# ndjinga/CirculantPreconditioner

Hardware: AMD Instinct MI355X
Metric: PCApply/s on 256^3 complex grid (higher is better)
Workload: dtype c128 (f64 complex); 1 GPU; 256x256x256 c128 circulant PCApply, transport symbol lambda=(0.6, 0.15, 0.02); global_batch=1, parallelism=single GPU

## Files before the change

### circulantpreconditioner_amd/_lib_ext.py

```python
from __future__ import annotations

import ctypes


class PetscScalar(ctypes.Structure):
    _fields_ = [("re", ctypes.c_double), ("im", ctypes.c_double)]

    @classmethod
    def of(cls, v) -> "PetscScalar":
        c = complex(v)
        return cls(c.real, c.imag)

    def __complex__(self):
        return complex(self.re, self.im)


class FFTPrecTransportContext(ctypes.Structure):
    _fields_ = [("spaceDim", ctypes.c_int64), ("n_x", ctypes.c_int64), ("n_y", ctypes.c_int64),
                ("n_z", ctypes.c_int64), ("lambda_x", PetscScalar), ("lambda_y", PetscScalar),
                ("lambda_z", PetscScalar), ("FFT_MAT", ctypes.c_void_p), ("intersectionMatrix", ctypes.c_void_p),
                ("Diag", ctypes.c_void_p), ("b_hat", ctypes.c_void_p), ("b_cartesien", ctypes.c_void_p)]


class StructuredTransportContext(ctypes.Structure):
# ... 42 lines not shown

class WaveResult(ctypes.Structure):
    _fields_ = [("steps", ctypes.c_int64), ("dt", ctypes.c_double), ("time", ctypes.c_double),
                ("total_its", ctypes.c_int64), ("max_step_its", ctypes.c_int64), ("min_step_its", ctypes.c_int64),
                ("last_reason", ctypes.c_int), ("all_converged", ctypes.c_int), ("last_residual", ctypes.c_double),
                ("last_norm_dU", ctypes.c_double), ("solve_seconds", ctypes.c_double),
                ("pc_seconds", ctypes.c_double), ("pc_calls", ctypes.c_int64), ("setup_seconds", ctypes.c_double),
                ("kappa", ctypes.c_double * 3), ("rstart", ctypes.c_int64), ("nlocal", ctypes.c_int64),
                ("loop_seconds", ctypes.c_double), ("dev_ms_", ctypes.c_double * 4),
                ("dev_launches_", ctypes.c_int64 * 4), ("fused_dots", ctypes.c_int64), ("fused_norms", ctypes.c_int64)]

    def as_dict(self) -> dict:
        d = {k: getattr(self, k) for k, _ in self._fields_ if k != "kappa" and not k.endswith("_")}
        d["kappa"] = list(self.kappa)
        d["dev_ms"] = dict(zip(("pcapply", "matmult", "vector", "copy"), self.dev_ms_))
        d["dev_launches"] = dict(zip(("pcapply", "matmult", "vector", "copy"), self.dev_launches_))
        return d


def declare(L) -> None:
    i64, dp, vp, c_int = ctypes.c_int64, ctypes.c_void_p, ctypes.c_void_p, ctypes.c_int
    S, P, cs = PetscScalar, ctypes.POINTER, ctypes.c_char_p
    sig = {
        "cfp_dist_get_unique_id": ([ctypes.c_char_p], c_int),
        "cfp_dist_unique_id_bytes": ([], c_int),
        "cfp_slab_layout": ([i64, i64, i64, c_int, c_int, P(i64)], c_int),
        "cfp_slab_work_size": ([i64, i64, i64, c_int, c_int, P(i64)], c_int),
        "cfp_slab_num_steps": ([i64, i64, i64, c_int, c_int, P(c_int)], c_int),
        "cfp_slab_step_info": ([i64, i64, i64, c_int, c_int, c_int, P(i64), P(ctypes.c_double)], c_int),
        "cfp_dist_plan_create": ([P(vp), i64, i64, i64, c_int, c_int, ctypes.c_char_p, c_int], c_int),
        "cfp_dist_plan_create_timeout": ([P(vp), i64, i64, i64, c_int, c_int, ctypes.c_char_p, c_int,
                                          ctypes.c_double], c_int),
        "cfp_dist_plan_rccl_info": ([vp, P(c_int), P(c_int), P(c_int), P(ctypes.c_double), ctypes.c_char_p, c_int],
                                    c_int),
        "cfp_rccl_version": ([P(c_int), ctypes.c_char_p, c_int], c_int),
        "cfp_rccl_blocking": ([P(c_int)], c_int),
        "cfp_dist_plan_destroy": ([vp], c_int),
        "cfp_dist_plan_create_external": ([P(vp), i64, i64, i64, c_int, c_int, c_int], c_int),
        "cfp_dist_plan_work_buffer": ([vp, P(ctypes.c_void_p)], c_int),
        "cfp_dist_plan_run_segment": ([vp, c_int, dp, dp, vp], c_int),
        "cfp_dist_plan_set_work_buffer": ([vp, dp], c_int),
        "cfp_dist_plan_set_symbol_transport": ([vp, dp], c_int),
        "cfp_dist_plan_apply": ([vp, dp, dp, vp], c_int),
        "cfp_dist_plan_profile_begin": ([vp, c_int, c_int], c_int),
        "cfp_dist_plan_profile_end": ([vp, dp, P(c_int)], c_int),
        "cfp_dist_plan_local_size": ([vp, P(i64)], c_int),
# ... 195 lines not shown
```

### circulantpreconditioner_amd/csrc/cfp_plan.hip

```cpp
#include <hip/hip_runtime.h>

#include <cmath>
#include <complex>
#include <cstdio>
#include <cstring>
#include <map>
#include <memory>
#include <mutex>
#include <string>
#include <vector>

#include "../../include/circulant_fft.h"
#include "cfp_blas.h"
#include "cfp_internal.h"
#include "cfp_host.h"
#include "cfp_three_pass.h"

using namespace cfp;

static thread_local std::string g_err;

namespace cfp {
int set_error(int code, const char* fmt, ...) {
  char buf[512];
// ... 35 lines not shown
  return CFP_SUCCESS;
}

namespace cfp {

std::vector<cd> host_twiddles(int n, int sign) {
  std::vector<cd> t((size_t)n);
  for (int k = 0; k < n; ++k) {
    long double a = 2.0L * 3.14159265358979323846264338327950288L * (long double)k / (long double)n;
    t[k] = make_cd((double)cosl(a), (double)(sign * sinl(a)));
  }
  return t;
}

std::vector<cd> host_transport_symbol(i64 n) {
  std::vector<cd> s((size_t)n, make_cd(0.0, 0.0));
  if (n <= 1) return s;
  for (i64 k = 0; k < n; ++k) {
    long double a = 2.0L * 3.14159265358979323846264338327950288L * (long double)k / (long double)n;
    s[k] = make_cd((double)(1.0L - cosl(a)), (double)sinl(a));
  }
  return s;
}

int ilog2_exact(i64 v) {
  if (v <= 0 || (v & (v - 1))) return -1;
  int l = 0;
  while ((1LL << l) < v) ++l;
  return l;
}

Side natural_side(int axis, const i64 n[3]) {
  Side s;
  const i64 nx = n[0], ny = n[1];
  s.seg_len = (int)n[axis];
  s.seg_shift = ilog2_exact(n[axis]);
  if (s.seg_shift < 0) s.seg_shift = 30;
  s.seg_stride = 0;
  if (axis == 0) { s.inner_stride = 0; s.outer_stride = nx; s.pt_stride = 1; }
  else if (axis == 1) { s.inner_stride = 1; s.outer_stride = nx * ny; s.pt_stride = nx; }
  else { s.inner_stride = 1; s.outer_stride = 0; s.pt_stride = nx * ny; }
  if (ilog2_exact(n[axis]) < 0) s.seg_shift = -1;
  return s;
}

void natural_cols(int axis, const i64 n[3], i64* ncols, i64* inner_n) {
// ... 12 lines not shown
  int sym_kind = 0;
  uint64_t sym_version = 0;
  cd* colsym = nullptr;
  cd* axsym = nullptr;
  cd* diag = nullptr;
  cd* host_stage = nullptr;
  cd* mid_buf = nullptr;
  double* post_partial = nullptr;
  cd* pre_buf = nullptr;
  struct GraphEntry {
    const cd* b;
    cd* x;
    hipGraphExec_t exec;
  };
  bool graph_on = false;
  hipStream_t cap_stream = nullptr;
  std::vector<GraphEntry> graphs;
  std::vector<int> axes;
  int fused_axis = 0;
  std::vector<cd> sym1d[3];
  i64 chunk_planes = 0;
  int schedule = CFP_SCHEDULE_AUTO;
  TPShape tp_shape;
  bool external_x = false;
  int split[3][2] = {{0, 0}, {0, 0}, {0, 0}};
  cd* tw4lo[3] = {nullptr, nullptr, nullptr};
  cd* tw4hi[3] = {nullptr, nullptr, nullptr};
  cd* possym[3] = {nullptr, nullptr, nullptr};
  bool long_axes() const { return split[0][0] || split[1][0] || split[2][0]; }
  std::vector<hipEvent_t> prof_ev;
  size_t prof_stride = 0, prof_cap = 0, prof_used = 0;
  size_t prof_every = 1, prof_calls = 0;
};

namespace cfp {
thread_local LaunchStamp g_stamp;
thread_local ApplyStamp g_apply_stamp;
}
extern "C" void cfp_apply_stamp_clear(void) { cfp::g_apply_stamp.start = cfp::g_apply_stamp.stop = nullptr; }

namespace {

struct DeviceGuard {
  int prev = -1;
  explicit DeviceGuard(int dev) {
    hipGetDevice(&prev);
// ... 12 lines not shown
  cd* d = nullptr;
  HIPCHK(hipMalloc(&d, sizeof(cd) * (size_t)n));
  HIPCHK(hipMemcpy(d, h.data(), sizeof(cd) * (size_t)n, hipMemcpyHostToDevice));
  p->tw[n] = d;
  return CFP_SUCCESS;
}

struct Step {
  int axis;
  int mode;
  bool from_b;
  bool scale;
  i64 z0, z1;
  int tp = -1;
  int sub = 0;
};

bool use_three_pass(const cfp_plan_s* p, bool diag_override) {
  const bool want = p->schedule == CFP_SCHEDULE_THREE_PASS ||
                    (p->schedule == CFP_SCHEDULE_AUTO && p->chunk_planes == 0 &&
                     (p->n[0] == 256 || p->n[0] == 128 || p->n[0] == 100 || p->n[0] == 512));
  if (!want || diag_override || p->sym_kind != 1 || p->external_x) return false;
  return three_pass_supported(p->n) || three_pass_sq_supported(p->n);
}

bool use_plane(const cfp_plan_s* p) {
  if (p->external_x || p->long_axes() || p->n[0] != p->n[1] || !plane_supported(p->n[0]) || p->n[2] < 2)
    return false;
  if (p->schedule == CFP_SCHEDULE_PLANE) return true;
  return p->schedule == CFP_SCHEDULE_AUTO && p->chunk_planes == 0 &&
         (p->n[0] == 100 || p->n[0] == 64 || p->n[0] == 32);
}

void order_axes(cfp_plan_s* p) {
  p->axes.clear();
  const int order_z[3] = {0, 1, 2}, order_y[3] = {0, 2, 1};
  const bool yf = p->schedule == CFP_SCHEDULE_FIVE_PASS_YFUSED ||
                  (p->schedule == CFP_SCHEDULE_AUTO && p->n[1] >= 512 && p->n[2] >= 512 && !three_pass_supported(p->n));
  const int* o = (yf && !p->long_axes()) ? order_y : order_z;
  std::vector<int> longs;
  for (int i = 0; i < 3; ++i) {
    if (p->n[o[i]] <= 1 || (p->external_x && o[i] == 0)) continue;
    if (p->split[o[i]][0]) longs.push_back(o[i]);
    else p->axes.push_back(o[i]);
  }
  p->fused_axis = p->axes.empty() ? (longs.empty() ? 0 : -1) : p->axes.back();
// ... 164 lines not shown
      if ((tn == 256 || tn == 512) && (p->tp_shape.mid == TP_MID_BLOCKED || p->tp_shape.mid == TP_MID_BLOCKED32)) {
        if (!p->mid_buf) HIPCHK(hipMalloc(&p->mid_buf, sizeof(cd) * (size_t)p->N));
        if (q.tp == 2) tin = p->mid_buf;
        else tout = p->mid_buf;
      }
      hipError_t e;
      if (fz && q.tp == 0 && fz->pre_cls) {
        a.pre_cls = fz->pre_cls;
        a.pre_cls_x = fz->pre_cls_x;
        a.pre_mask = fz->pre_mask;
        a.pre_tab = fz->pre_tab;
        a.pre_nd = fz->pre_nd;
        a.pre_ncls = fz->pre_ncls;
        for (int k = 0; k < 3; ++k) a.pre_off[k] = fz->pre_off[k];
        e = launch_three_pass_fused(0, tn, tin, tout, a, s, nullptr);
      } else if (fz && q.tp == 2 && fz->post_nv > 0) {
        for (int j = 0; j < TP_POST_MAX; ++j) a.post_v[j] = fz->post_v[j];
        a.post_nv = fz->post_nv;
        a.post_self = fz->post_self;
        a.post_partial = fz->post_partial;
        e = launch_three_pass_fused(2, tn, tin, tout, a, s, p3grid);
      } else {
        a.krylov = fz != nullptr || g_apply_stamp.start != nullptr;
        e = launch_three_pass(q.tp, tn, tin, tout, a, p->tp_shape, s);
      }
      g_stamp = LaunchStamp{};
      if (e != hipSuccess) return hip_error(e, "3-sweep launch");
      continue;
    }
    if (q.sub == 4) {
      const int pn = (int)p->n[0];
      int prc = ensure_tw(p, pn);
      if (prc) return prc;
      if (ev) HIPCHK(hipEventRecord((*ev)[2 * i], s));
      hipError_t e = launch_plane_pass(q.mode == PASS_PLANE_INV, pn, p->n[2], q.from_b ? b : x, x, p->tw[pn],
                                       q.scale ? invN : 1.0, s);
      if (e != hipSuccess) return hip_error(e, "plane pass launch");
      if (ev) HIPCHK(hipEventRecord((*ev)[2 * i + 1], s));
      continue;
    }
    if (q.sub == 3) {
      if (ev) HIPCHK(hipEventRecord((*ev)[2 * i], s));
      hipError_t e = launch_sym_divide_positions(x, p->possym[0], p->possym[1], p->possym[2], p->n[0], p->n[1],
                                                 p->n[2], s);
      if (e != hipSuccess) return hip_error(e, "symbol divide");
      if (ev) HIPCHK(hipEventRecord((*ev)[2 * i + 1], s));
// ... 102 lines not shown
  free_symbol(p);
  HIPCHK(hipMalloc(&p->colsym, sizeof(cd) * (size_t)ncols));
  HIPCHK(hipMalloc(&p->axsym, sizeof(cd) * (size_t)nf));
  HIPCHK(hipMemcpy(p->colsym, col.data(), sizeof(cd) * (size_t)ncols, hipMemcpyHostToDevice));
  HIPCHK(hipMemcpy(p->axsym, ax.data(), sizeof(cd) * (size_t)nf, hipMemcpyHostToDevice));
  for (int a = 0; a < 3; ++a) p->sym1d[a] = s_nat[a];
  p->sym_kind = 1;
  return CFP_SUCCESS;
}

int set_separable(cfp_plan_s* p, const std::vector<cd> hat[3], const double lam[6]) {
  std::vector<cd> s[3];
  for (int a = 0; a < 3; ++a) {
    std::complex<double> l = lamc(lam, a);
    s[a].resize(hat[a].size());
    for (size_t k = 0; k < hat[a].size(); ++k) {
      std::complex<double> c(hat[a][k].x, hat[a][k].y);
      const double re = c.real() * l.real() - c.imag() * l.imag();
      const double im = c.real() * l.imag() + c.imag() * l.real();
      s[a][k] = make_cd(re, im);
    }
  }
  ++p->sym_version;
  return upload_separable(p, s);
}

}

extern "C" int cfp_plan_create(cfp_plan_t* plan, int64_t nx, int64_t ny, int64_t nz, int device) {
  if (!plan) return set_error(CFP_ERR_ARG_NULL, "plan is NULL");
  *plan = nullptr;
  if (nx < 1 || ny < 1 || nz < 1) return set_error(CFP_ERR_ARG_OUTOFRANGE, "grid sizes must be >= 1");
  const int64_t dims_in[3] = {nx, ny, nz};
  int split[3][2] = {{0, 0}, {0, 0}, {0, 0}};
  for (int a = 0; a < 3; ++a) {
    if (dims_in[a] <= 4096) continue;
    i64 best = 0;
    for (i64 d = 2; d <= 4096; ++d)
      if (dims_in[a] % d == 0 && dims_in[a] / d <= 4096) {
        const i64 o = dims_in[a] / d;
        if (best == 0 || std::llabs(d - o) < std::llabs(best - dims_in[a] / best)) best = d;
      }
    if (best == 0)
      return set_error(CFP_ERR_SUP, "axis length %lld is not a product of two factors <= 4096", (long long)dims_in[a]);
    split[a][0] = (int)best;
    split[a][1] = (int)(dims_in[a] / best);
  }
  int ndev = 0;
// ... 51 lines not shown
  }
  if (p->host_stage) hipFree(p->host_stage);
  if (p->mid_buf) hipFree(p->mid_buf);
  if (p->post_partial) hipFree(p->post_partial);
  if (p->pre_buf) hipFree(p->pre_buf);
  graph_clear(p);
  if (p->cap_stream) hipStreamDestroy(p->cap_stream);
  for (auto& e : p->prof_ev) hipEventDestroy(e);
  delete p;
  return CFP_SUCCESS;
}

extern "C" int cfp_plan_symbol_version(cfp_plan_t p, uint64_t* version) {
  if (!p || !version) return set_error(CFP_ERR_ARG_NULL, "NULL argument");
  *version = p->sym_version;
  return CFP_SUCCESS;
}

extern "C" int cfp_plan_set_symbol_transport(cfp_plan_t p, const double lam[6]) {
  if (!p || !lam) return set_error(CFP_ERR_ARG_NULL, "NULL argument");
  DeviceGuard dg(p->device);
  std::vector<cd> hat[3];
  for (int a = 0; a < 3; ++a) hat[a] = host_transport_symbol(p->n[a]);
  return set_separable(p, hat, lam);
}

extern "C" int cfp_plan_set_symbol_separable(cfp_plan_t p, const double* cx, const double* cy, const double* cz,
                                             const double lam[6]) {
  if (!p || !cx || !cy || !cz || !lam) return set_error(CFP_ERR_ARG_NULL, "NULL argument");
  DeviceGuard dg(p->device);
  std::vector<cd> hat[3];
  const double* src[3] = {cx, cy, cz};
  for (int a = 0; a < 3; ++a) {
    hat[a].resize((size_t)p->n[a]);
    std::memcpy(hat[a].data(), src[a], sizeof(cd) * (size_t)p->n[a]);
  }
  return set_separable(p, hat, lam);
}

extern "C" int cfp_plan_set_diag(cfp_plan_t p, const double* diag, int on_device) {
  if (!p || !diag) return set_error(CFP_ERR_ARG_NULL, "NULL argument");
  if (p->long_axes()) return set_error(CFP_ERR_SUP, "an explicit Diag needs axes <= 4096 (use a separable symbol)");
  DeviceGuard dg(p->device);
  free_symbol(p);
  ++p->sym_version;
  HIPCHK(hipMalloc(&p->diag, sizeof(cd) * (size_t)p->N));
  HIPCHK(hipMemcpy(p->diag, diag, sizeof(cd) * (size_t)p->N, on_device ? hipMemcpyDeviceToDevice : hipMemcpyHostToDevice));
  p->sym_kind = 2;
  return CFP_SUCCESS;
}

extern "C" int cfp_plan_get_diag(cfp_plan_t p, double* diag_dev, void* stream) {
  if (!p || !diag_dev) return set_error(CFP_ERR_ARG_NULL, "NULL argument");
  DeviceGuard dg(p->device);
  hipStream_t s = (hipStream_t)stream;
  if (p->sym_kind == 2) {
    HIPCHK(hipMemcpyAsync(diag_dev, p->diag, sizeof(cd) * (size_t)p->N, hipMemcpyDeviceToDevice, s));
    return CFP_SUCCESS;
  }
  if (p->sym_kind != 1) return set_error(CFP_ERR_ARG_WRONGSTATE, "no symbol set");
  cd* tmp[3] = {nullptr, nullptr, nullptr};
  for (int a = 0; a < 3; ++a) {
    HIPCHK(hipMalloc(&tmp[a], sizeof(cd) * (size_t)p->n[a]));
    HIPCHK(hipMemcpy(tmp[a], p->sym1d[a].data(), sizeof(cd) * (size_t)p->n[a], hipMemcpyHostToDevice));
  }
  const cd one = make_cd(1.0, 0.0);
  hipError_t e = launch_build_diag_separable((cd*)diag_dev, tmp[0], tmp[1], tmp[2], p->n[0], p->n[1], p->n[2], one,
                                             one, one, s);
// ... 398 lines not shown
```

### circulantpreconditioner_amd/csrc/cfp_three_pass.h

```cpp
#pragma once
#include "cfp_internal.h"

namespace cfp {

#ifndef CFP_ROWS_XCD
#define CFP_ROWS_XCD 1
#endif

struct TPArgs {
  const cd* tw;
  const cd* colsym;
  const cd* axsym;
  double scale;
  int lnyl = 0;
  i64 chunk = 0;
  int k1_off = 0;
  const unsigned char* pre_cls = nullptr;
  const unsigned char* pre_cls_x = nullptr;
  const unsigned char* pre_mask = nullptr;
  const cd* pre_tab = nullptr;
  int pre_nd = 0, pre_ncls = 0;
  int pre_off[3] = {0, 0, 0};
  const cd* post_v[4] = {nullptr, nullptr, nullptr, nullptr};
  int post_nv = 0;
  int post_self = 0;
  double* post_partial = nullptr;
  int krylov = 0;
};


enum { TP_MID_DEFAULT = 0, TP_MID_LANE64 = 1, TP_MID_LANE32 = 2, TP_MID_SWAP64 = 3, TP_MID_SWAP64_PF = 4,
       TP_MID_BLOCKED = 5, TP_MID_BLOCKED32 = 6, TP_MID_SWAP32X = 7, TP_MID_ROWSALT = 8 };
struct TPShape {
  int n1 = 0;
  int mid = 0;
};

#define TP_PRE_MAX_CLS 16
#define TP_POST_MAX 4
bool three_pass_fused_supported(int n, TPShape shape);
hipError_t launch_three_pass_fused(int stage, int n, const cd* in, cd* out, const TPArgs& a, hipStream_t s,
                                   unsigned* grid_out);

bool three_pass_supported(const i64 n[3]);
bool three_pass_sq_supported(const i64 n[3]);
hipError_t launch_three_pass_sq(int stage, int n, const cd* in, cd* out, const TPArgs& a, TPShape shape,
                                hipStream_t s);
bool three_pass_shape_valid(int n1, int mid, i64 n = 0);
hipError_t launch_three_pass(int stage, int n, const cd* in, cd* out, const TPArgs& a, TPShape shape,
                             hipStream_t s);
bool three_pass_slab_supported(const i64 n[3], int P);
int three_pass_slab_n2(i64 n);
hipError_t launch_three_pass_slab(int stage, int n, const cd* in, cd* out, const TPArgs& a, int nzl, hipStream_t s);
hipError_t launch_three_pass_real(int stage, int n, const double* b, cd* H, cd* Q, double* x, const TPArgs& a,
                                  hipStream_t s, bool alt_rows = false);

struct WTPArgs {
  const cd* tw;
  WaveSym wave;
  double scale;
  const cd* post_v[4] = {nullptr, nullptr, nullptr, nullptr};
  int post_nv = 0, post_self = 0;
  double* post_partial = nullptr;
};
bool wave_three_pass_supported(const i64 n[3], int ncomp);
// ... 5 lines not shown
```

### circulantpreconditioner_amd/csrc/cfp_three_pass.hip

```cpp
#include "cfp_fft_device.h"
#include "cfp_lane.h"
#include "cfp_three_pass.h"

#include <hip/hip_ext.h>

#ifndef CFP_REAL_MID_XCD
#define CFP_REAL_MID_XCD 1
#endif

#define TP_LAUNCH(K, G, B, S, ...)                                                                    \
  do {                                                                                                \
    if (g_stamp.start || g_stamp.stop)                                                                \
      hipExtLaunchKernelGGL(K, G, B, 0, S, g_stamp.start, g_stamp.stop, 0, __VA_ARGS__);              \
    else                                                                                              \
      hipLaunchKernelGGL(K, G, B, 0, S, __VA_ARGS__);                                                 \
  } while (0)

namespace cfp {

namespace {

__device__ __forceinline__ cd dft4_dif(cd v, int q) {
  const cd p = dpp_c<DPP_XOR2>(v);
  cd t = (q & 2) ? csub(p, v) : cadd(v, p);
// ... 683 lines not shown
    if constexpr (PF) {
      lds_barrier();
      if (it + (int)gridDim.x < nunits) prefetch(XCD ? xcd_unit(it + gridDim.x, gridDim.x) : it + (int)gridDim.x);
    }
    stage_b(v);
    {
      const int c = idx(c0), tz = idx(tz0);
      const cd w = tw_y(u, c);
      cd* dst = col_ptr(u, c, tz);
      if constexpr (PROBE & PR_NO_STORE) {
        double acc = 0.0;
#pragma unroll
        for (int m = 0; m < 16; ++m) acc += v[m].x * w.x + v[m].y;
        if (acc == 1.2345e300) dst[0] = make_cd(acc, 0.0);
      } else {
#pragma unroll
        for (int m = 0; m < 16; ++m) gstore<ST>(dst + zs * TZ * m, cconj(cmul(v[m], w)));
      }
    }
    if constexpr (!PF) lds_barrier();
  }
}


bool three_pass_supported(const i64 n[3]) {
  return n[0] == n[1] && n[1] == n[2] && (n[0] == 128 || n[0] == 256 || n[0] == 512);
}

static int cu_count() {
  static int cus = 0;
  if (!cus) {
    int dev = 0;
    if (hipGetDevice(&dev) != hipSuccess ||
        hipDeviceGetAttribute(&cus, hipDeviceAttributeMultiprocessorCount, dev) != hipSuccess || cus < 1)
      cus = 256;
  }
  return cus;
}

static unsigned grid_of(int units, int per_cu) {
  const int g = per_cu * cu_count();
  return (unsigned)(units < g ? units : g);
}
static unsigned grid_xcd(int units, int per_cu) {
  unsigned g = grid_of(units, per_cu), p = 1;
  while (2 * p <= g) p *= 2;
// ... 276 lines not shown
  else launch_rows<N1, TN, PER_CU, PTS, XS, LP, 0, XCD, P1F, P3F, kRowsWave>(stage, in, out, a, s);
}

template <int T, int N2, int TN, int PER_CU, int PTS = 16, bool XS = true>
static void launch_mid(cd* data, const TPArgs& a, hipStream_t s) {
  constexpr int units = (TN / (T / N2)) * (TN / N2);
  TP_LAUNCH((k_tp_mid<0, T, N2, TN, PTS, XS>), dim3(grid_of(units, PER_CU)), dim3(T * (TN / PTS)), s, data, a, units);
}

template <int N2, int TN, bool PF = false, bool BL = false, int T = 64>
static void launch_mid_sw(cd* data, const TPArgs& a, hipStream_t s) {
  constexpr int units = (TN / (T / N2)) * (TN / N2);
  if constexpr (T == 64 && N2 == 8 && TN == 256 && PF && !BL) {
    if (a.krylov) {
      TP_LAUNCH((k_tp_mid_sw<T, N2, TN, 0, PF, TN, 0, kP2LoadFlags, BL, false, 1>), dim3(grid_of(units, 64 / T)),
                dim3(T * (TN / 16)), s, data, a, units);
      return;
    }
  }
  TP_LAUNCH((k_tp_mid_sw<T, N2, TN, 0, PF, TN, 0, kP2LoadFlags, BL>), dim3(grid_of(units, 64 / T)),
            dim3(T * (TN / 16)), s, data, a, units);
}

bool three_pass_slab_supported(const i64 n[3], int P) {
  const bool cube = n[0] == n[1] && n[1] == n[2] && (n[0] == 256 || n[0] == 512);
  return cube && P >= 1 && P <= 16 && (32 % P) == 0;
}

int three_pass_slab_n2(i64 n) { return n == 512 ? 16 : 8; }

hipError_t launch_three_pass_slab(int stage, int n, const cd* in, cd* out, const TPArgs& a, int nzl, hipStream_t s) {
  if (n == 512) {
    constexpr int W = kRowsWave ? F_WAVE_LDS : 0;
    if (stage == 1) {
      const int nk1 = (1 << a.lnyl) / 16;
      const int units = 256 * nk1;
      const unsigned g = grid_xcd(units, 1);
      if (g) TP_LAUNCH((k_tp_mid<0, 32, 16, 512, 16, true, 512, true>), dim3(g), dim3(1024), s, out, a, units);
      else TP_LAUNCH((k_tp_mid<0, 32, 16, 512, 16, true, 512, false>), dim3(grid_of(units, 1)), dim3(1024), s, out, a,
                     units);
    } else {
      const int units = nzl * 16;
      const unsigned gx = kRowsXCD && units >= (int)grid_of(1 << 30, 1) ? grid_xcd(units, 1) : 0;
      const unsigned g = gx ? gx : grid_of(units, 1);
      if (stage == 0 && gx)
        TP_LAUNCH((k_tp_rows<false, F_NT_LD | W, 32, 512, 16, true, kRowsLP, 0, true>), dim3(g), dim3(1024), s, in, out, a, units);
// ... 45 lines not shown
    TP_LAUNCH((k_tp_rows<false, kP1Flags | W, 32, 256, 16, true, kRowsLP, 0, XCD, 0, 1>), dim3(g), dim3(512), s, in,
              out, a, units);
  else
    TP_LAUNCH((k_tp_rows<true, kP3Flags | W, 32, 256, 16, true, kRowsLP, 0, XCD, 0, TP_POST_MAX>), dim3(g), dim3(512),
              s, in, out, a, units);
}

hipError_t launch_three_pass_fused(int stage, int n, const cd* in, cd* out, const TPArgs& a, hipStream_t s,
                                   unsigned* grid_out) {
  if (n != 256 || (stage != 0 && stage != 2)) return hipErrorNotSupported;
  if (stage == 0 && (!a.pre_cls || in == out || a.pre_ncls < 1 || a.pre_ncls > TP_PRE_MAX_CLS || a.pre_nd < 1 ||
                     a.pre_nd > 3))
    return hipErrorInvalidValue;
  if (stage == 2 && (a.post_nv < 1 || a.post_nv > TP_POST_MAX || !a.post_partial)) return hipErrorInvalidValue;
  constexpr int units = 256 * 8;
  const unsigned gx = kRowsXCD ? grid_xcd(units, 2) : 0;
  const unsigned g = gx ? gx : grid_of(units, 2);
  if (grid_out) *grid_out = g;
  if (gx) launch_rows_fused<true>(stage, in, out, a, s, g);
  else launch_rows_fused<false>(stage, in, out, a, s, g);
  return hipGetLastError();
}

bool three_pass_shape_valid(int n1, int mid, i64 n) {
  if (mid == TP_MID_ROWSALT) return n1 == 0;
  if (n1 == 16) return n == 128 && mid >= TP_MID_DEFAULT && mid <= TP_MID_SWAP64;
  return (n1 == 0 || n1 == 32 || n1 == 64) && (mid >= 0 && mid <= TP_MID_SWAP32X) &&
         !(mid >= TP_MID_BLOCKED && n1 == 64);
}

hipError_t launch_three_pass(int stage, int n, const cd* in, cd* out, const TPArgs& a, TPShape shape,
                             hipStream_t s) {
  const bool ra = shape.mid == TP_MID_ROWSALT;
  if (ra) shape.mid = TP_MID_DEFAULT;
  if (n == 100) return launch_three_pass_sq(stage, n, in, out, a, shape, s);
  if (n == 512) {
    const bool bl = shape.mid == TP_MID_BLOCKED, bl8 = shape.mid == TP_MID_BLOCKED32;
    if (stage == 1) {
      constexpr int units = (512 / 2) * 32;
      const unsigned g = grid_xcd(units, 1);
      if (g == 0) return hipErrorNotSupported;
      if (bl) TP_LAUNCH((k_tp_mid<0, 32, 16, 512, 16, true, 512, true, 2>), dim3(g), dim3(1024), s, out, a, units);
      else if (bl8) TP_LAUNCH((k_tp_mid<0, 32, 16, 512, 16, true, 512, true, 8>), dim3(g), dim3(1024), s, out, a, units);
      else TP_LAUNCH((k_tp_mid<0, 32, 16, 512, 16, true, 512, true>), dim3(g), dim3(1024), s, out, a, units);
    } else if (bl) {
      launch_rows<32, 512, 1, 16, true, kRowsLP, 2, true>(stage, in, out, a, s);
// ... 46 lines not shown
  if (shape.mid == TP_MID_SWAP32X) {
    if (stage != 1) {
      launch_rows<32, 256, 2, 16, true, kRowsLP>(stage, in, out, a, s);
    } else {
      constexpr int units = (256 / 4) * 32;
      const unsigned g = grid_xcd(units, 2);
      if (g == 0) return hipErrorNotSupported;
      if (pf_ok)
        TP_LAUNCH((k_tp_mid_sw<32, 8, 256, 0, true, 256, 0, kP2LoadFlags, false, true>), dim3(g), dim3(512), s, out, a,
                  units);
      else
        TP_LAUNCH((k_tp_mid_sw<32, 8, 256, 0, false, 256, 0, kP2LoadFlags, false, true>), dim3(g), dim3(512), s, out, a,
                  units);
    }
    return hipGetLastError();
  }
  if (shape.mid == TP_MID_BLOCKED32) {
    if (stage != 1) launch_rows<32, 256, 2, 16, true, kRowsLP, 4, true>(stage, in, out, a, s);
    else if (pf_ok) launch_mid_sw<8, 256, true, true, 32>(out, a, s);
    else launch_mid_sw<8, 256, false, true, 32>(out, a, s);
    return hipGetLastError();
  }
  if (stage == 1) {
    if ((shape.mid == TP_MID_SWAP64_PF || shape.mid == TP_MID_DEFAULT) && pf_ok) {
      if (n1 == 64) launch_mid_sw<4, 256, true>(out, a, s);
      else launch_mid_sw<8, 256, true>(out, a, s);
    } else if (shape.mid == TP_MID_SWAP64 || shape.mid == TP_MID_SWAP64_PF || shape.mid == TP_MID_DEFAULT) {
      if (n1 == 64) launch_mid_sw<4, 256>(out, a, s);
      else launch_mid_sw<8, 256>(out, a, s);
    } else if (n1 == 64) {
      if (t32) launch_mid<32, 4, 256, 2>(out, a, s);
      else launch_mid<64, 4, 256, 1>(out, a, s);
    } else if (t32) {
      launch_mid<32, 8, 256, 2>(out, a, s);
    } else {
      launch_mid<64, 8, 256, 1>(out, a, s);
    }
  } else if (n1 == 64) {
    launch_rows<64, 256, 1>(stage, in, out, a, s);
  } else {
    launch_rows_ab<32, 256, 2, 16, true, kRowsLP>(ra, stage, in, out, a, s);
  }
  return hipGetLastError();
}

}
```

### circulantpreconditioner_amd/plan.py

```python
from __future__ import annotations

import ctypes
from typing import Sequence

import numpy as np
import torch

from . import _lib
from ._lib import check, lib


def _stream_handle(stream=None) -> int:
    if stream is None:
        stream = torch.cuda.current_stream()
    return int(stream.cuda_stream)


def _dev_ptr(t: torch.Tensor, n: int, name: str, device: int | None = None) -> int:
    if not isinstance(t, torch.Tensor):
        raise TypeError(f"{name} must be a torch.Tensor")
    if t.dtype != torch.complex128:
        raise TypeError(f"{name} must be complex128, got {t.dtype}")
    if not t.is_cuda:
        raise ValueError(f"{name} must be a device (HIP) tensor")
# ... 181 lines not shown
        return self

    TP_MIDS = {"default": 0, "lane64": 1, "lane32": 2, "swap64": 3, "swap64pf": 4, "blocked": 5, "blocked32": 6,
               "swap32x": 7, "rowsalt": 8}

    def set_three_pass_shape(self, n1: int = 0, mid: str | int = "default") -> "CirculantPlan":
        m = self.TP_MIDS[mid] if isinstance(mid, str) else int(mid)
        check(lib().cfp_plan_set_three_pass_shape(self._h, int(n1), m))
        return self

    def passes(self) -> list:
        n = ctypes.c_int()
        check(lib().cfp_plan_num_passes(self._h, ctypes.byref(n)))
        out = []
        for i in range(n.value):
            ax, nn, mode, fast = ctypes.c_int(), ctypes.c_int(), ctypes.c_int(), ctypes.c_int()
            nc = ctypes.c_int64()
            check(lib().cfp_plan_pass_info(self._h, i, ctypes.byref(ax), ctypes.byref(nn), ctypes.byref(nc),
                                           ctypes.byref(mode), ctypes.byref(fast)))
            out.append({"axis": PASS_AXES[ax.value], "n": nn.value, "ncols": nc.value,
                        "mode": PASS_MODES[mode.value], "fast": bool(fast.value)})
        return out

    def time_passes(self, b: torch.Tensor, x: torch.Tensor, iters: int = 20, stream=None) -> list:
        npass = len(self.passes())
        ms = (ctypes.c_double * npass)()
        check(lib().cfp_plan_time_passes(self._h, _dev_ptr(b, self.N, "b", self.device),
                                         _dev_ptr(x, self.N, "x", self.device), int(iters),
                                         ms, _stream_handle(stream)))
        return list(ms)

    def profile_begin(self, max_applies: int, every: int = 1) -> "CirculantPlan":
        check(lib().cfp_plan_profile_begin(self._h, int(max_applies), int(every)))
        return self

    def profile_end(self) -> tuple:
        npass = len(self.passes())
        ms = (ctypes.c_double * npass)()
        n = ctypes.c_int()
        check(lib().cfp_plan_profile_end(self._h, ms, ctypes.byref(n)))
        return list(ms), n.value

    def close(self) -> None:
        if getattr(self, "_h", None) is not None and self._h.value:
            lib().cfp_plan_destroy(self._h)
            self._h = None
# ... 115 lines not shown
```

### include/circulant_fft.h

```cpp
#ifndef CIRCULANT_FFT_H
#define CIRCULANT_FFT_H

#include <stddef.h>
#include <stdint.h>

#ifdef __cplusplus
extern "C" {
#endif

#define CFP_SUCCESS 0
#define CFP_ERR_MEM 55
#define CFP_ERR_SUP 56
#define CFP_ERR_ARG_SIZ 60
#define CFP_ERR_ARG_WRONG 62
#define CFP_ERR_ARG_OUTOFRANGE 63
#define CFP_ERR_ARG_WRONGSTATE 73
#define CFP_ERR_LIB 76
#define CFP_ERR_ARG_NULL 85

typedef struct cfp_plan_s *cfp_plan_t;

const char *cfp_version(void);
const char *cfp_last_error(void);
int cfp_device_count(int *count);
// ... 33 lines not shown
} cfp_apply_ex_t;
int cfp_plan_apply_ex(cfp_plan_t plan, const double *b_dev, double *x_dev, void *stream, cfp_apply_ex_t *ex);
int cfp_plan_apply_ex_fusable(cfp_plan_t plan, const cfp_stencil_t *pre, int post_nv, int *fusable);

int cfp_plan_forward(cfp_plan_t plan, const double *in_dev, double *out_dev, void *stream);
int cfp_plan_backward(cfp_plan_t plan, const double *in_dev, double *out_dev, void *stream);

int cfp_plan_set_chunking(cfp_plan_t plan, int64_t chunk_planes);

int cfp_plan_set_graph(cfp_plan_t plan, int on);

#define CFP_SCHEDULE_AUTO 0
#define CFP_SCHEDULE_FIVE_PASS 1
#define CFP_SCHEDULE_THREE_PASS 2
#define CFP_SCHEDULE_FIVE_PASS_YFUSED 3
#define CFP_SCHEDULE_PLANE 4
int cfp_plan_set_schedule(cfp_plan_t plan, int schedule);
#define CFP_TP_MID_DEFAULT 0
#define CFP_TP_MID_LANE64 1
#define CFP_TP_MID_LANE32 2
#define CFP_TP_MID_SWAP64 3
#define CFP_TP_MID_SWAP64_PF 4
int cfp_plan_set_three_pass_shape(cfp_plan_t plan, int n1, int mid);

int cfp_plan_num_passes(cfp_plan_t plan, int *passes);
int cfp_plan_pass_info(cfp_plan_t plan, int pass, int *axis, int *n, int64_t *ncols, int *mode, int *fast);
int cfp_plan_time_passes(cfp_plan_t plan, const double *b_dev, double *x_dev, int iters, double *ms_out,
                         void *stream);
int cfp_plan_profile_begin(cfp_plan_t plan, int max_applies, int every);
int cfp_plan_profile_end(cfp_plan_t plan, double *ms_out, int *applies);

int cfp_pointwise_divide(double *w_dev, const double *x_dev, const double *y_dev, int64_t n, void *stream);
int cfp_scale(double *x_dev, double alpha_re, double alpha_im, int64_t n, void *stream);
int cfp_fill_uniform(double *x_dev, int64_t n, uint64_t seed, int64_t offset, void *stream);
int cfp_build_diag_3d(double *diag_dev, const double *cx_hat_dev, const double *cy_hat_dev,
                      const double *cz_hat_dev, int64_t nx, int64_t ny, int64_t nz, const double lam[6],
                      void *stream);
int cfp_transport_symbol_1d(int64_t n, double *out_host);

#ifdef __cplusplus
}
#endif
#endif
```

Before: 3363 PCApply/s.

## Replace z-axis FFT-divide-IFFT in three-pass mid stage with cyclic recurrence solve

For the transport symbol on a 256^3 grid, the middle pass no longer does a forward z FFT, a divide by the symbol and an inverse z FFT. It solves the z-direction circulant bidiagonal system directly with a parallel first-order linear recurrence. The recurrence uses lane shuffles, an LDS carry across waves and a closed-form wraparound correction. It is only enabled when a host check shows the ratio |lambda_z|/|denominator| stays below 1, which keeps the recurrence stable. The aim is to cut the arithmetic of the z transforms, at the cost of a specialized, numerically conditioned code path limited to one grid size and shape.

```diff
diff --git a/circulantpreconditioner_amd/_lib_ext.py b/circulantpreconditioner_amd/_lib_ext.py
--- a/circulantpreconditioner_amd/_lib_ext.py
+++ b/circulantpreconditioner_amd/_lib_ext.py
@@ -88,6 +88,7 @@
     i64, dp, vp, c_int = ctypes.c_int64, ctypes.c_void_p, ctypes.c_void_p, ctypes.c_int
     S, P, cs = PetscScalar, ctypes.POINTER, ctypes.c_char_p
     sig = {
+        "cfp_plan_mid_kernel": ([vp, P(c_int)], c_int), "cfp_transport_z_ratio": ([i64, i64, dp, P(ctypes.c_double)], c_int),
         "cfp_dist_get_unique_id": ([ctypes.c_char_p], c_int),
         "cfp_dist_unique_id_bytes": ([], c_int),
         "cfp_slab_layout": ([i64, i64, i64, c_int, c_int, P(i64)], c_int),
diff --git a/circulantpreconditioner_amd/csrc/cfp_plan.hip b/circulantpreconditioner_amd/csrc/cfp_plan.hip
--- a/circulantpreconditioner_amd/csrc/cfp_plan.hip
+++ b/circulantpreconditioner_amd/csrc/cfp_plan.hip
@@ -81,6 +81,20 @@
   }
   return s;
 }
+
+double transport_z_ratio(const std::vector<cd>& sx, const std::vector<cd>& sy, std::complex<double> lz) {
+  double amax = 0.0;
+  const double lzn = std::abs(lz);
+  for (const cd& y : sy)
+    for (const cd& x : sx) {
+      const std::complex<double> den(x.x + y.x + 1.0 + lz.real(), x.y + y.y + lz.imag());
+      const double d = std::abs(den);
+      const double r = d > 0.0 ? lzn / d : (lzn > 0.0 ? INFINITY : 0.0);
+      if (!(r <= amax)) amax = r;
+    }
+  return amax;
+}
+constexpr double kZrecMaxRatio = 1.0 - 1.0 / 8192.0;
 
 int ilog2_exact(i64 v) {
   if (v <= 0 || (v & (v - 1))) return -1;
@@ -139,6 +153,9 @@
   i64 chunk_planes = 0;
   int schedule = CFP_SCHEDULE_AUTO;
   TPShape tp_shape;
+  bool zrec_ok = false;
+  double zrec_amax = 0.0;
+  cd lamz = cfp::make_cd(0.0, 0.0);
   bool external_x = false;
   int split[3][2] = {{0, 0}, {0, 0}, {0, 0}};
   cd* tw4lo[3] = {nullptr, nullptr, nullptr};
@@ -197,6 +214,10 @@
                      (p->n[0] == 256 || p->n[0] == 128 || p->n[0] == 100 || p->n[0] == 512));
   if (!want || diag_override || p->sym_kind != 1 || p->external_x) return false;
   return three_pass_supported(p->n) || three_pass_sq_supported(p->n);
+}
+bool plan_zrec(const cfp_plan_s* p) {
+  return p->zrec_ok && p->sym_kind == 1 && p->fused_axis == 2 && use_three_pass(p, false) &&
+         three_pass_zrec_shape((int)p->n[0], p->tp_shape);
 }
 
 bool use_plane(const cfp_plan_s* p) {
@@ -407,6 +428,10 @@
         e = launch_three_pass_fused(2, tn, tin, tout, a, s, p3grid);
       } else {
         a.krylov = fz != nullptr || g_apply_stamp.start != nullptr;
+        if (q.tp == 1 && plan_zrec(p)) {
+          a.zrec = 1;
+          a.lamz = p->lamz;
+        }
         e = launch_three_pass(q.tp, tn, tin, tout, a, p->tp_shape, s);
       }
       g_stamp = LaunchStamp{};
@@ -555,8 +580,10 @@
     }
   }
   ++p->sym_version;
+  p->zrec_ok = false;
   return upload_separable(p, s);
 }
+
 
 }
 
@@ -654,7 +681,34 @@
   DeviceGuard dg(p->device);
   std::vector<cd> hat[3];
   for (int a = 0; a < 3; ++a) hat[a] = host_transport_symbol(p->n[a]);
-  return set_separable(p, hat, lam);
+  int rc = set_separable(p, hat, lam);
+  if (rc) return rc;
+  if (p->n[0] == 256 && p->n[1] == 256 && p->n[2] == 256) {
+    const std::complex<double> lz = lamc(lam, 2);
+    p->zrec_amax = transport_z_ratio(p->sym1d[0], p->sym1d[1], lz);
+    p->zrec_ok = p->zrec_amax <= kZrecMaxRatio;
+    p->lamz = make_cd(lz.real(), lz.imag());
+  }
+  return CFP_SUCCESS;
+}
+
+extern "C" int cfp_plan_mid_kernel(cfp_plan_t p, int* kind) {
+  if (!p || !kind) return set_error(CFP_ERR_ARG_NULL, "NULL argument");
+  *kind = plan_zrec(p) ? 1 : 0;
+  return CFP_SUCCESS;
+}
+
+extern "C" int cfp_transport_z_ratio(int64_t nx, int64_t ny, const double lam[6], double* amax) {
+  if (!lam || !amax) return set_error(CFP_ERR_ARG_NULL, "NULL argument");
+  if (nx < 1 || ny < 1) return set_error(CFP_ERR_ARG_OUTOFRANGE, "grid sizes must be >= 1");
+  std::vector<cd> s[2] = {host_transport_symbol(nx), host_transport_symbol(ny)};
+  for (int a = 0; a < 2; ++a)
+    for (cd& v : s[a]) {
+      const std::complex<double> t = std::complex<double>(v.x, v.y) * lamc(lam, a);
+      v = make_cd(t.real(), t.imag());
+    }
+  *amax = transport_z_ratio(s[0], s[1], lamc(lam, 2));
+  return CFP_SUCCESS;
 }
 
 extern "C" int cfp_plan_set_symbol_separable(cfp_plan_t p, const double* cx, const double* cy, const double* cz,
@@ -676,6 +730,7 @@
   DeviceGuard dg(p->device);
   free_symbol(p);
   ++p->sym_version;
+  p->zrec_ok = false;
   HIPCHK(hipMalloc(&p->diag, sizeof(cd) * (size_t)p->N));
   HIPCHK(hipMemcpy(p->diag, diag, sizeof(cd) * (size_t)p->N, on_device ? hipMemcpyDeviceToDevice : hipMemcpyHostToDevice));
   p->sym_kind = 2;
diff --git a/circulantpreconditioner_amd/csrc/cfp_three_pass.h b/circulantpreconditioner_amd/csrc/cfp_three_pass.h
--- a/circulantpreconditioner_amd/csrc/cfp_three_pass.h
+++ b/circulantpreconditioner_amd/csrc/cfp_three_pass.h
@@ -26,6 +26,8 @@
   int post_self = 0;
   double* post_partial = nullptr;
   int krylov = 0;
+  int zrec = 0;
+  cd lamz = make_cd(0.0, 0.0);
 };
 
 
@@ -41,6 +43,8 @@
 bool three_pass_fused_supported(int n, TPShape shape);
 hipError_t launch_three_pass_fused(int stage, int n, const cd* in, cd* out, const TPArgs& a, hipStream_t s,
                                    unsigned* grid_out);
+
+bool three_pass_zrec_shape(int n, TPShape shape);
 
 bool three_pass_supported(const i64 n[3]);
 bool three_pass_sq_supported(const i64 n[3]);
diff --git a/circulantpreconditioner_amd/csrc/cfp_three_pass.hip b/circulantpreconditioner_amd/csrc/cfp_three_pass.hip
--- a/circulantpreconditioner_amd/csrc/cfp_three_pass.hip
+++ b/circulantpreconditioner_amd/csrc/cfp_three_pass.hip
@@ -729,6 +729,243 @@
   }
 }
 
+constexpr int kRecNPF = 7;
+template <int PROBE, bool PF, int LD>
+__device__ __forceinline__ void tp_mid_rec_body(cd* __restrict__ data, const TPArgs& a, int nunits,
+                                                double* __restrict__ pf_l, cd* __restrict__ carr,
+                                                cd* __restrict__ ctab, cd* __restrict__ tw_l) {
+  constexpr int TN = 256, N2 = 8, N1 = TN / N2, XT = 8, NXT = TN / XT, NW = 16;
+  constexpr int NPF = PF ? kRecNPF : 0;
+  const int tid = threadIdx.x;
+  const int lane = tid & 63, x = lane & 7, zl = lane >> 3;
+  const int wv = __builtin_amdgcn_readfirstlane(tid / 64);
+  const i64 zs = (i64)TN << (a.lnyl ? a.lnyl : ilog2(TN));
+  const cd lz = a.lamz;
+  const auto idx = [](int i) {
+    asm volatile("" : "+v"(i));
+    return i;
+  };
+  const auto colsym_of = [&](int u) {
+    return a.colsym[(u % NXT) * XT + x + (i64)TN * (a.k1_off + u / NXT + N1 * zl)];
+  };
+  const auto ctab_put = [&](int buf, cd cs) {
+    const cd den = make_cd(cs.x + 1.0 + lz.x, cs.y + lz.y);
+    const double id = 1.0 / fma(den.x, den.x, den.y * den.y);
+    const cd ri = make_cd(den.x * id, -den.y * id);
+    ctab[(2 * buf) * 64 + idx(lane)] = cmul(lz, ri);
+    ctab[(2 * buf + 1) * 64 + idx(lane)] = make_cd(ri.x * (double)TN, ri.y * (double)TN);
+  };
+  if (tid < TN) tw_l[tid] = a.tw[tid];
+  if (wv == 0 && (int)blockIdx.x < nunits) ctab_put(0, colsym_of((int)blockIdx.x));
+  __syncthreads();
+  const unsigned loff = 16u * ((unsigned)x + (unsigned)zs * 2u * (unsigned)zl);
+  const auto slot_ptr = [&](int u, int m) {
+    return data + ((u % NXT) * XT + (i64)TN * (N2 * (u / NXT) + (m & 7)) + zs * (16 * wv + (m >> 3)));
+  };
+  const auto at = [](cd* base, unsigned off) { return reinterpret_cast<cd*>(reinterpret_cast<char*>(base) + off); };
+  const auto prefetch = [&](int u) {
+    unsigned lo0 = loff;
+    asm volatile("" : "+s"(u), "+v"(lo0));
+#pragma unroll
+    for (int m = 0; m < NPF; ++m)
+      __builtin_amdgcn_global_load_lds((glb_void_t*)at(slot_ptr(u, m), lo0), (lds_void_t*)(pf_l + (wv * NPF + m) * 128),
+                                       16, 0, (LD & F_NT_LD) ? 2 : 0);
+  };
+  if constexpr (PF) {
+    if ((int)blockIdx.x < nunits) prefetch((int)blockIdx.x);
+  }
+  const bool up3 = (zl & 1) != 0, up4 = (zl & 2) != 0, up5 = (zl & 4) != 0;
+  const cd zero = make_cd(0.0, 0.0), one = make_cd(1.0, 0.0);
+  const auto pin = [](cd& w) { asm volatile("" : "+v"(w.x), "+v"(w.y)); };
+  const auto cfma = [](cd p, cd q, cd c) {
+    return make_cd(fma(p.x, q.x, fma(-p.y, q.y, c.x)), fma(p.x, q.y, fma(p.y, q.x, c.y)));
+  };
+
+  int par = 0, buf = 0;
+  const auto unit = [&](const int it, auto more_c) {
+    constexpr bool more = decltype(more_c)::value;
+    const int u = it;
+    const int k1 = a.k1_off + u / NXT;
+    const int nbuf = buf == 2 ? 0 : buf + 1;
+    cd v[16], csn = zero;
+    if constexpr (PROBE & PR_NO_LOAD) {
+#pragma unroll
+      for (int m = 0; m < 16; ++m) v[m] = make_cd(lane + m, wv + u);
+    } else {
+      if constexpr (PF) {
+        asm volatile("s_waitcnt vmcnt(0)" ::: "memory");
+#pragma unroll
+        for (int m = 0; m < NPF; ++m)
+          v[m] = fromv(*reinterpret_cast<const dv2*>(pf_l + (wv * NPF + m) * 128 + 2 * idx(lane)));
+      }
+      if constexpr (more) csn = colsym_of(it + (int)gridDim.x);
+      {
+        int ul = u;
+        unsigned lo1 = loff;
+        asm volatile("" : "+s"(ul), "+v"(lo1));
+#pragma unroll
+        for (int m = NPF; m < 16; ++m) v[m] = gload<LD>(at(slot_ptr(ul, m), lo1));
+      }
+    }
+    if (more && wv == 0) ctab_put(nbuf, csn);
+#pragma unroll
+    for (int y = 1; y < N2; ++y) {
+      const cd w = tw_l[(y * k1) & (TN - 1)];
+      v[y] = cmul(v[y], w);
+      v[8 + y] = cmul(v[8 + y], w);
+    }
+    if constexpr (PF && more && !(PROBE & PR_NO_LOAD)) {
+#pragma unroll
+      for (int m = 0; m < 16; ++m) pin(v[m]);
+      prefetch(it + (int)gridDim.x);
+    }
+    __builtin_amdgcn_sched_barrier(0);
+    if constexpr (!(PROBE & PR_NO_Y2)) {
+      dft_reg<8>(v);
+#pragma unroll
+      for (int m = 0; m < 8; ++m) pin(v[m]);
+      __builtin_amdgcn_sched_barrier(0);
+      dft_reg<8>(v + 8);
+#pragma unroll
+      for (int m = 8; m < 16; ++m) pin(v[m]);
+      __builtin_amdgcn_sched_barrier(0);
+    }
+    if constexpr (!(PROBE & PR_NO_ZMATH)) {
+      const auto pow2zl = [&](cd aa) {
+        cd pw = cmul(aa, aa), q = up3 ? pw : one;
+        pw = cmul(pw, pw);
+        q = up4 ? cmul(q, pw) : q;
+        pw = cmul(pw, pw);
+        return up5 ? cmul(q, pw) : q;
+      };
+#pragma unroll
+      for (int k2 = 0; k2 < 8; ++k2) {
+        const int c = (idx(lane) & 7) + 8 * k2;
+        const cd aa = ctab[(2 * buf) * 64 + c], r = ctab[(2 * buf + 1) * 64 + c];
+        const cd v0 = cmul(v[k2], r), v1 = cmul(v[8 + k2], r);
+        cd S = cfma(aa, v0, v1), X, lo, hi, pw = cmul(aa, aa), q;
+        __builtin_amdgcn_sched_barrier(0);
+        {
+          const cd pr = lane_xor8(S);
+          lo = up3 ? pr : S;
+          hi = up3 ? S : pr;
+          X = up3 ? lo : zero;
+          S = cfma(pw, lo, hi);
+          q = up3 ? pw : one;
+          pw = cmul(pw, pw);
+        }
+        __builtin_amdgcn_sched_barrier(0);
+        {
+          lo = S;
+          hi = S;
+          swap_c<4>(lo, hi);
+          if (up4) X = cfma(q, lo, X);
+          S = cfma(pw, lo, hi);
+          q = up4 ? cmul(q, pw) : q;
+          pw = cmul(pw, pw);
+        }
+        __builtin_amdgcn_sched_barrier(0);
+        {
+          lo = S;
+          hi = S;
+          swap_c<5>(lo, hi);
+          if (up5) X = cfma(q, lo, X);
+          S = cfma(pw, lo, hi);
+        }
+        v[k2] = cfma(aa, X, v0);
+        v[8 + k2] = cfma(aa, v[k2], v1);
+        pin(v[k2]);
+        pin(v[8 + k2]);
+        if (zl == k2) carr[(par * NW + wv) * 64 + idx(lane)] = S;
+        __builtin_amdgcn_sched_barrier(0);
+      }
+      lds_barrier();
+      cd cin;
+      {
+        const int ln = idx(lane);
+        const cd am = ctab[(2 * buf) * 64 + ln];
+        const cd am2 = cmul(am, am), am4 = cmul(am2, am2), am8 = cmul(am4, am4);
+        const cd A = cmul(am8, am8);
+        cd acc = carr[(par * NW + wv) * 64 + ln];
+#pragma unroll
+        for (int k = 14; k >= 0; --k) {
+          acc = cfma(acc, A, carr[(par * NW + ((wv - 1 - k) & 15)) * 64 + ln]);
+          if ((k & 3) == 0) __builtin_amdgcn_sched_barrier(0);
+        }
+        const cd A2 = cmul(A, A), A4 = cmul(A2, A2), A8 = cmul(A4, A4), A16 = cmul(A8, A8);
+        const cd d = make_cd(1.0 - A16.x, -A16.y);
+        const double id = 1.0 / fma(d.x, d.x, d.y * d.y);
+        cin = make_cd(fma(acc.x, d.x, acc.y * d.y) * id, fma(acc.y, d.x, -acc.x * d.y) * id);
+      }
+#pragma unroll
+      for (int k2 = 0; k2 < 8; ++k2) {
+        const int c = (idx(lane) & 7) + 8 * k2;
+        const long long bx = __double_as_longlong(cin.x), by = __double_as_longlong(cin.y);
+        const unsigned xl = (unsigned)__builtin_amdgcn_ds_bpermute(4 * c, (int)(bx & 0xffffffffll));
+        const unsigned xh = (unsigned)__builtin_amdgcn_ds_bpermute(4 * c, (int)(bx >> 32));
+        const unsigned yl = (unsigned)__builtin_amdgcn_ds_bpermute(4 * c, (int)(by & 0xffffffffll));
+        const unsigned yh = (unsigned)__builtin_amdgcn_ds_bpermute(4 * c, (int)(by >> 32));
+        const cd ci = make_cd(__longlong_as_double((long long)(((unsigned long long)xh << 32) | xl)),
+                              __longlong_as_double((long long)(((unsigned long long)yh << 32) | yl)));
+        const cd aa = ctab[(2 * buf) * 64 + c];
+        const cd g = cmul(cmul(aa, pow2zl(aa)), ci);
+        v[k2] = cadd(v[k2], g);
+        v[8 + k2] = cfma(aa, g, v[8 + k2]);
+        pin(v[k2]);
+        pin(v[8 + k2]);
+        __builtin_amdgcn_sched_barrier(0);
+      }
+    }
+#pragma unroll
+    for (int m = 0; m < 16; ++m) v[m] = cconj(v[m]);
+    if constexpr (!(PROBE & PR_NO_Y2)) {
+      dft_reg<8>(v);
+#pragma unroll
+      for (int m = 0; m < 8; ++m) pin(v[m]);
+      __builtin_amdgcn_sched_barrier(0);
+      dft_reg<8>(v + 8);
+#pragma unroll
+      for (int m = 8; m < 16; ++m) pin(v[m]);
+      __builtin_amdgcn_sched_barrier(0);
+    }
+    {
+      int k1s = k1, us = u;
+      unsigned lo2 = loff;
+      asm volatile("" : "+s"(k1s), "+s"(us), "+v"(lo2));
+      if constexpr (PROBE & PR_NO_STORE) {
+        double acc = 0.0;
+#pragma unroll
+        for (int m = 0; m < 16; ++m) acc += v[m].x + v[m].y;
+        if (acc == 1.2345e300) *at(slot_ptr(us, 0), lo2) = make_cd(acc, 0.0);
+      } else {
+#pragma unroll
+        for (int m = 0; m < 16; ++m) {
+          const cd w = (m & 7) ? tw_l[((m & 7) * k1s) & (TN - 1)] : one;
+          gstore<0>(at(slot_ptr(us, m), lo2), cconj(cmul(v[m], w)));
+        }
+      }
+    }
+    par ^= 1;
+    buf = nbuf;
+  };
+  int it = blockIdx.x;
+  for (; it + (int)gridDim.x < nunits; it += gridDim.x) unit(it, std::true_type{});
+  if (it < nunits) unit(it, std::false_type{});
+}
+
+template <int PROBE = 0, bool PF = false, int LD = 0, int TAG = 0>
+__global__ void __launch_bounds__(1024) __attribute__((amdgpu_waves_per_eu(4)))
+k_tp_mid_rec(cd* data, TPArgs a, int nunits) {
+#ifndef CFP_KEXP
+  static_assert(PROBE == 0, "timing probes are built in tools/kexp only");
+#endif
+  __shared__ __attribute__((aligned(16))) double pf_l[PF ? 16 * kRecNPF * 128 : 2];
+  __shared__ __attribute__((aligned(16))) cd carr[2 * 16 * 64];
+  __shared__ __attribute__((aligned(16))) cd ctab[3 * 2 * 64];
+  __shared__ cd tw_l[256];
+  tp_mid_rec_body<PROBE, PF, LD>(data, a, nunits, pf_l, carr, ctab, tw_l);
+}
+
 
 bool three_pass_supported(const i64 n[3]) {
   return n[0] == n[1] && n[1] == n[2] && (n[0] == 128 || n[0] == 256 || n[0] == 512);
@@ -1051,6 +1288,15 @@
             dim3(T * (TN / 16)), s, data, a, units);
 }
 
+template <bool PF>
+static void launch_mid_rec(cd* data, const TPArgs& a, hipStream_t s) {
+  constexpr int units = (256 / 8) * (256 / 8);
+  if (a.krylov)
+    TP_LAUNCH((k_tp_mid_rec<0, PF, kP2LoadFlags, 1>), dim3(grid_of(units, 1)), dim3(1024), s, data, a, units);
+  else
+    TP_LAUNCH((k_tp_mid_rec<0, PF, kP2LoadFlags>), dim3(grid_of(units, 1)), dim3(1024), s, data, a, units);
+}
+
 bool three_pass_slab_supported(const i64 n[3], int P) {
   const bool cube = n[0] == n[1] && n[1] == n[2] && (n[0] == 256 || n[0] == 512);
   return cube && P >= 1 && P <= 16 && (32 % P) == 0;
@@ -1142,6 +1388,10 @@
   return hipGetLastError();
 }
 
+bool three_pass_zrec_shape(int n, TPShape shape) {
+  return n == 256 && shape.mid == TP_MID_DEFAULT && (shape.n1 == 0 || shape.n1 == 32);
+}
+
 bool three_pass_shape_valid(int n1, int mid, i64 n) {
   if (mid == TP_MID_ROWSALT) return n1 == 0;
   if (n1 == 16) return n == 128 && mid >= TP_MID_DEFAULT && mid <= TP_MID_SWAP64;
@@ -1234,7 +1484,10 @@
     return hipGetLastError();
   }
   if (stage == 1) {
-    if ((shape.mid == TP_MID_SWAP64_PF || shape.mid == TP_MID_DEFAULT) && pf_ok) {
+    if (a.zrec && three_pass_zrec_shape(n, shape)) {
+      if (pf_ok) launch_mid_rec<true>(out, a, s);
+      else launch_mid_rec<false>(out, a, s);
+    } else if ((shape.mid == TP_MID_SWAP64_PF || shape.mid == TP_MID_DEFAULT) && pf_ok) {
       if (n1 == 64) launch_mid_sw<4, 256, true>(out, a, s);
       else launch_mid_sw<8, 256, true>(out, a, s);
     } else if (shape.mid == TP_MID_SWAP64 || shape.mid == TP_MID_SWAP64_PF || shape.mid == TP_MID_DEFAULT) {
diff --git a/circulantpreconditioner_amd/plan.py b/circulantpreconditioner_amd/plan.py
--- a/circulantpreconditioner_amd/plan.py
+++ b/circulantpreconditioner_amd/plan.py
@@ -227,6 +227,11 @@
                         "mode": PASS_MODES[mode.value], "fast": bool(fast.value)})
         return out
 
+    def mid_kernel(self) -> str:
+        k = ctypes.c_int()
+        check(lib().cfp_plan_mid_kernel(self._h, ctypes.byref(k)))
+        return "zrec" if k.value == 1 else "fft"
+
     def time_passes(self, b: torch.Tensor, x: torch.Tensor, iters: int = 20, stream=None) -> list:
         npass = len(self.passes())
         ms = (ctypes.c_double * npass)()
diff --git a/include/circulant_fft.h b/include/circulant_fft.h
--- a/include/circulant_fft.h
+++ b/include/circulant_fft.h
@@ -79,6 +79,9 @@
 #define CFP_TP_MID_SWAP64 3
 #define CFP_TP_MID_SWAP64_PF 4
 int cfp_plan_set_three_pass_shape(cfp_plan_t plan, int n1, int mid);
+#define CFP_MID_KERNEL_FFT 0
+#define CFP_MID_KERNEL_ZREC 1
+int cfp_plan_mid_kernel(cfp_plan_t plan, int *kind);
 
 int cfp_plan_num_passes(cfp_plan_t plan, int *passes);
 int cfp_plan_pass_info(cfp_plan_t plan, int pass, int *axis, int *n, int64_t *ncols, int *mode, int *fast);
@@ -94,6 +97,7 @@
                       const double *cz_hat_dev, int64_t nx, int64_t ny, int64_t nz, const double lam[6],
                       void *stream);
 int cfp_transport_symbol_1d(int64_t n, double *out_host);
+int cfp_transport_z_ratio(int64_t nx, int64_t ny, const double lam[6], double *amax_host);
 
 #ifdef __cplusplus
 }
```

Result: faster. 3591 PCApply/s (median of 6 runs) (+6.8%).
